# gsneha26/SegAlign

Hardware: AMD Instinct MI355X
Metric: Gbp query seeded+filtered+extended per sec (higher is better)
Workload: dtype int32

## Files before the change

### segalign_amd/csrc/extend.hip

```cpp
#include <atomic>
#include <cstdlib>

#include "kernels.h"
#include "kmer_dev.h"

namespace sa {

constexpr int EXT_THREADS = 256;
constexpr int NEG = -(1 << 26);
constexpr int DEAD = -(1 << 29);
constexpr uint64_t TERM_ALL = 0x4040404040404040ull;
constexpr uint32_t BIAS = SEQ_PAD;

__device__ __forceinline__ int f64_to_i32(double x) { return (int)x; }

enum : int { PH_RIGHT = 0, PH_LEFT = 1, PH_FIN = 2, PH_IDLE = 3 };

template <int CTRL, int ROW_MASK = 0xf, int BANK_MASK = 0xf>
__device__ __forceinline__ int dpp_mov(int old, int v) {
    return __builtin_amdgcn_update_dpp(old, v, CTRL, ROW_MASK, BANK_MASK, false);
}
__device__ __forceinline__ uint32_t wave_inclusive_sum(uint32_t v) {
    v += (uint32_t)dpp_mov<0x111>(0, (int)v);
    v += (uint32_t)dpp_mov<0x112>(0, (int)v);
// ... 410 lines not shown
        if (threadIdx.x < L2_NSUB) {
            raw = a.l2_count[threadIdx.x * L2_CNT_STRIDE];
            s_l2cnt[threadIdx.x & (SRC == SRC_CAND ? 0xFFFF : 0)] = min(raw, a.l2_cap);
        }
        __syncthreads();
        if (threadIdx.x <= L2_NSUB) {
            uint32_t pre = 0;
            for (int t = 0; t < (int)threadIdx.x; t++) pre += s_l2cnt[t & (SRC == SRC_CAND ? 0xFFFF : 0)];
            s_l2pre[threadIdx.x & (SRC == SRC_CAND ? 0xFFFF : 0)] = pre;
            if (blockIdx.x == 0 && threadIdx.x == L2_NSUB) *a.l2_total = pre;
        }
        if (blockIdx.x == 0 && threadIdx.x < L2_NSUB) {
            uint32_t mx = raw;
            for (int o = 32; o >= 1; o >>= 1) mx = max(mx, (uint32_t)__shfl_xor((int)mx, o, 64));
            if ((threadIdx.x & 63) == 0) atomicMax(a.l2_max, mx);
        }
    }
    __syncthreads();
    CandRec* stage = s_cand[threadIdx.x >> 6];
    int n_stage = 0;

    const int lane = threadIdx.x & 63;
    const unsigned long long lane_lt = (1ull << lane) - 1ull;
    const int xdrop = a.xdrop;
    const int fin_batch = a.fin_batch;
    const uint32_t long_cap = a.long_cap;

    const uint64_t total_hits = SRC == SRC_CAND ? (uint64_t)s_l2pre[SRC == SRC_CAND ? L2_NSUB : 0] : a.num_hits;
    const uint64_t num_buf = (total_hits + 63) >> 6;
    const uint64_t W = (uint64_t)gridDim.x * (PK_THREADS / 64);
    const uint64_t wid = (uint64_t)__builtin_amdgcn_readfirstlane((int)(blockIdx.x * (PK_THREADS / 64) + (threadIdx.x >> 6)));
    const uint64_t G = TD ? 1ull : W;
    const uint64_t buf_end = TD ? ((wid + 1) * num_buf) / W : num_buf;
    uint64_t cur_buf = TD ? (wid * num_buf) / W : wid;
    uint64_t nxt_buf = cur_buf + G;
    auto buf_count = [&](uint64_t b) -> int {
        if (b >= buf_end) return 0;
        uint64_t rem = total_hits - (b << 6);
        return rem >= 64 ? 64 : (int)rem;
    };
    TdCursor cursor = {0u, {0u, 0u, 0ull}, 0u};
    if (TD && cur_buf < buf_end) cursor.seek(a, lane, (uint32_t)(cur_buf << 6));
    uint32_t f_idx = 0;
    uint32_t f_known = 0, f_tm = 0, f_flags = 3;
    auto fetch = [&](uint64_t b, int cnt) -> Hit {
        Hit h = {0u, 0u};
        f_idx = (uint32_t)(b << 6) + (uint32_t)lane;
        if (SRC == SRC_HITS) {
            if (lane < cnt) h = a.hits[(b << 6) + lane];
        } else if (SRC == SRC_CAND) {
            if (lane < cnt) {
                const uint32_t g = (uint32_t)(b << 6) + (uint32_t)lane;
                uint32_t sl = 0;
#pragma unroll
                for (uint32_t step = L2_NSUB / 2; step >= 1; step >>= 1)
                    if (s_l2pre[(sl + step) & (SRC == SRC_CAND ? 0xFFFFu : 0u)] <= g) sl += step;
                const L2Rec c = a.l2_list[(size_t)sl * a.l2_cap + (g - s_l2pre[sl & (SRC == SRC_CAND ? 0xFFFFu : 0u)])];
                h.ref_loc = c.ref_loc;
                h.query_loc = c.query_loc;
                f_idx = c.hidx;
                f_known = c.meta & 0xFFFFu;
                f_flags = (c.meta >> 16) & 3u;
                const int t16 = (int)c.state >> 16;
                f_tm = ((uint32_t)t16 & 0xFFFFu) | ((uint32_t)(t16 + (int)(c.state & 0xFFFFu)) << 16);
            }
        } else if (cnt > 0) {
            uint64_t entry;
            uint32_t qp;
            cursor.locate(a, lane, (uint32_t)(b << 6), entry, qp);
            if (lane < cnt) {
                h.ref_loc = a.td_pos[entry] + a.seed_size;
                h.query_loc = qp + a.seed_size;
            }
        }
        return h;
    };
    int buf_cnt = buf_count(cur_buf), nxt_cnt = buf_count(nxt_buf), consumed = 0;
    Hit buf = fetch(cur_buf, buf_cnt);
    uint32_t buf_idx = f_idx, buf_known = f_known, buf_tm = f_tm, buf_flags = f_flags;
    Hit nxt = fetch(nxt_buf, nxt_cnt);
    uint32_t nxt_idx = f_idx, nxt_known = f_known, nxt_tm = f_tm, nxt_flags = f_flags;

    int phase = PH_FIN;
    bool has_hit = false, forward = false;
    uint32_t ref_loc = 0, query_loc = 0, hidx = 0;
    uint32_t walked = 0;
    uint4 h_tw = {0u, 0u, 0u, 0u}, h_qlo = {0u, 0u, 0u, 0u}, h_qhi = {0u, 0u, 0u, 0u};
    s16x2 T = {0, 0}, M = {0, 0};
    int bestR = 0, best = 0;
    bool left_known = false;
    int left_best = 0;

    for (;;) {
        if (phase < PH_FIN) {
            const bool left = phase == PH_LEFT;
            uint4 qlo, qhi, tw;
            if (left && walked == 0u) {
                qlo = h_qlo; qhi = h_qhi; tw = h_tw;
            } else {
                const int32_t qpos = left ? (int32_t)query_loc - (int32_t)walked : (int32_t)(query_loc + walked);
                const int32_t qbyte = left ? (qpos >> 1) - 32 : (qpos >> 1);
                const uint8_t* qp = a.query4 + (size_t)(qpos & 1) * a.query4_stride + qbyte;
                qlo = load16u(qp);
                qhi = load16u(qp + 16);
                const int32_t tpos = left ? (int32_t)ref_loc - (int32_t)walked : (int32_t)(ref_loc + walked);
                const int32_t tbyte = left ? (tpos >> 2) - 16 : (tpos >> 2);
                const bool fresh = !left && walked == 0u;
                const uint32_t jj0 = (uint32_t)(tbyte + PACK2_BIAS);
                const uint32_t line = (fresh ? jj0 - 16u : jj0) / (uint32_t)PACK2_PAYLOAD;
                const uint8_t* tp = a.ref2 + (size_t)(tpos & 3) * a.ref2_stride + (jj0 + 32u * line);
                tw = load16u(tp);
                if (fresh) {
                    h_tw = load16u(tp - 16);
                    h_qlo = load16u(qp - 32);
                    h_qhi = load16u(qp - 16);
                }
            }
            uint32_t tw0, tw1, tw2, tw3, qw0, qw1, qw2, qw3, qw4, qw5, qw6, qw7;
            if (left) {
                const uint32_t R = 0x00010203u, D = 0x88888888u;
                qw0 = __builtin_amdgcn_perm(0u, qhi.w, R) | D; qw1 = __builtin_amdgcn_perm(0u, qhi.z, R) | D;
                qw2 = __builtin_amdgcn_perm(0u, qhi.y, R) | D; qw3 = __builtin_amdgcn_perm(0u, qhi.x, R) | D;
                qw4 = __builtin_amdgcn_perm(0u, qlo.w, R) | D; qw5 = __builtin_amdgcn_perm(0u, qlo.z, R) | D;
                qw6 = __builtin_amdgcn_perm(0u, qlo.y, R) | D; qw7 = __builtin_amdgcn_perm(0u, qlo.x, R) | D;
                tw0 = __builtin_bitreverse32(tw.w); tw1 = __builtin_bitreverse32(tw.z);
                tw2 = __builtin_bitreverse32(tw.y); tw3 = __builtin_bitreverse32(tw.x);
            } else {
                qw0 = qlo.x; qw1 = qlo.y; qw2 = qlo.z; qw3 = qlo.w; qw4 = qhi.x; qw5 = qhi.y; qw6 = qhi.z; qw7 = qhi.w;
                tw0 = tw.x; tw1 = tw.y; tw2 = tw.z; tw3 = tw.w;
            }
            bool alive = true;
            int m = 0;
#pragma unroll
            for (int st = 0; st < 4; st++) {
                if (alive) {
                    const uint32_t td = st == 0 ? tw0 : st == 1 ? tw1 : st == 2 ? tw2 : tw3;
                    const uint32_t q0 = st == 0 ? qw0 : st == 1 ? qw2 : st == 2 ? qw4 : qw6;
                    const uint32_t q1 = st == 0 ? qw1 : st == 1 ? qw3 : st == 2 ? qw5 : qw7;
#pragma unroll
                    for (int j = 0; j < 8; j++) {
                        const uint32_t qd = j < 4 ? q0 : q1;
                        uint32_t qaddr;
                        switch (j & 3) {
                            case 0: asm("v_lshlrev_b32_sdwa %0, %1, %2 dst_sel:DWORD dst_unused:UNUSED_PAD src0_sel:DWORD src1_sel:BYTE_0" : "=v"(qaddr) : "v"(6), "v"(qd)); break;
                            case 1: asm("v_lshlrev_b32_sdwa %0, %1, %2 dst_sel:DWORD dst_unused:UNUSED_PAD src0_sel:DWORD src1_sel:BYTE_1" : "=v"(qaddr) : "v"(6), "v"(qd)); break;
                            case 2: asm("v_lshlrev_b32_sdwa %0, %1, %2 dst_sel:DWORD dst_unused:UNUSED_PAD src0_sel:DWORD src1_sel:BYTE_2" : "=v"(qaddr) : "v"(6), "v"(qd)); break;
                            default: asm("v_lshlrev_b32_sdwa %0, %1, %2 dst_sel:DWORD dst_unused:UNUSED_PAD src0_sel:DWORD src1_sel:BYTE_3" : "=v"(qaddr) : "v"(6), "v"(qd)); break;
                        }
                        const uint32_t rp = (td >> (4 * j)) & 15u;
                        const uint32_t addr = (rp << 2) | qaddr;
                        const s16x2 e = __builtin_bit_cast(s16x2, *reinterpret_cast<const uint32_t*>(reinterpret_cast<const char*>(s_pk) + addr));
                        const s16x2 Tb = T.yy;
                        T = __builtin_elementwise_add_sat(Tb, e);
                        M = __builtin_elementwise_max(M, T);
                    }
                    m = max((int)M.x, (int)M.y);
                    alive = (m - (int)T.y) <= xdrop;
                }
            }
            walked += 64;
            if (!alive) {
                if (!left) {
                    bestR = m;
                    if (SRC == SRC_CAND && left_known) {
                        best = left_best;
                        phase = PH_FIN;
                    } else {
                        phase = PH_LEFT;
                        walked = 0;
                        T = (s16x2){0, 0};
                        M = (s16x2){0, 0};
                    }
                } else {
                    best = m;
                    phase = PH_FIN;
                }
            } else if (walked + (uint32_t)(64 - CTX_R_BASES) >= long_cap) {
                forward = true;
                phase = PH_FIN;
            }
        }

        const unsigned long long fin = __ballot(phase == PH_FIN);
        const unsigned long long live = __ballot(phase < PH_FIN);
        if (fin != 0ull && (__popcll(fin) >= fin_batch || live == 0ull)) {
            bool cand = false;
            if (phase == PH_FIN && has_hit) cand = forward || bound_passes(a, bestR + best);
            {
                CandRec cr;
                cr.ref_loc = ref_loc; cr.query_loc = query_loc; cr.hidx = hidx;
                stage_append(stage, n_stage, cand, cr, a.cand_list, a.cand_count, a.cand_cap_recs, lane, lane_lt);
            }
            if (a.audit_list) {
                uint2 ar;
                ar.x = ref_loc; ar.y = query_loc;
                wave_append(phase == PH_FIN && has_hit && !cand, ar, a.audit_list, a.audit_count, a.audit_cap, lane, lane_lt);
            }
            unsigned long long need = fin;
            bool got = false;
            Hit mine = {0u, 0u};
            uint32_t mine_idx = 0, mine_known = 0, mine_tm = 0, mine_flags = 3;
            while (need != 0ull) {
                const int avail = buf_cnt - consumed;
                if (avail <= 0) {
                    if (nxt_cnt == 0) break;
                    buf = nxt;
                    buf_idx = nxt_idx;
                    buf_known = nxt_known; buf_tm = nxt_tm; buf_flags = nxt_flags;
                    buf_cnt = nxt_cnt;
                    cur_buf = nxt_buf;
                    consumed = 0;
                    nxt_buf += G;
                    nxt_cnt = buf_count(nxt_buf);
                    nxt = fetch(nxt_buf, nxt_cnt);
                    nxt_idx = f_idx;
                    nxt_known = f_known; nxt_tm = f_tm; nxt_flags = f_flags;
                    continue;
                }
                const int rank = __popcll(need & lane_lt);
                const bool take = ((need >> lane) & 1ull) && rank < avail;
                const int src = (consumed + rank) & 63;
                const uint32_t hr = (uint32_t)__shfl((int)buf.ref_loc, src, 64);
                const uint32_t hq = (uint32_t)__shfl((int)buf.query_loc, src, 64);
                const uint32_t hi = SRC == SRC_CAND ? (uint32_t)__shfl((int)buf_idx, src, 64) : (uint32_t)(cur_buf << 6) + (uint32_t)src;
                uint32_t hk = 0, ht = 0, hf = 3;
                if (SRC == SRC_CAND) {
                    hk = (uint32_t)__shfl((int)buf_known, src, 64);
                    ht = (uint32_t)__shfl((int)buf_tm, src, 64);
                    hf = (uint32_t)__shfl((int)buf_flags, src, 64);
                }
                if (take) {
                    mine.ref_loc = hr;
                    mine.query_loc = hq;
                    mine_idx = hi;
                    mine_known = hk; mine_tm = ht; mine_flags = hf;
                    got = true;
                }
                consumed += min(__popcll(need), avail);
                need &= ~__ballot(take);
            }
            if (phase == PH_FIN) {
                forward = false;
                if (got) {
                    has_hit = true;
                    ref_loc = mine.ref_loc;
                    query_loc = mine.query_loc;
                    hidx = mine_idx;
                    bestR = 0;
                    best = 0;
                    bool skip = false;
                    if (a.rm) skip = !(ref_loc >= a.rm_win_start && ref_loc <= a.rm_win_end);
                    left_known = false;
                    if (skip || ref_loc > a.ref_len || query_loc > a.query_len) {
                        phase = PH_FIN;
                    } else if (SRC == SRC_CAND && mine_flags == 0u) {
                        bestR = (int)mine_known;
                        best = (int)mine_tm;
                        phase = PH_FIN;
                    } else if (SRC == SRC_CAND && mine_flags == 2u) {
                        bestR = (int)mine_known;
                        phase = PH_LEFT;
                        walked = (uint32_t)CTX_L_BASES + a.left_skip;
                        const short t16 = (short)(mine_tm & 0xFFFFu), m16 = (short)(mine_tm >> 16);
                        T = (s16x2){t16, t16};
                        M = (s16x2){m16, m16};
                    } else {
                        phase = PH_RIGHT;
                        walked = 0;
                        T = (s16x2){0, 0};
                        M = (s16x2){0, 0};
                        if (SRC == SRC_CAND && mine_flags == 1u) {
                            left_known = true;
                            left_best = (int)mine_known;
                            if (a.l2_right_state) {
                                walked = (uint32_t)CTX_R_BASES;
                                const short t16 = (short)(mine_tm & 0xFFFFu), m16 = (short)(mine_tm >> 16);
                                T = (s16x2){t16, t16};
                                M = (s16x2){m16, m16};
                            }
                        }
                    }
                } else {
                    has_hit = false;
                    phase = PH_IDLE;
                }
            }
        }
        if (__ballot(phase != PH_IDLE) == 0ull) break;
    }
    stage_flush(stage, n_stage, a.cand_list, a.cand_count, a.cand_cap_recs, lane);
}

constexpr int CTX_THREADS = 1024;
constexpr int CTX_THREADS_MAX = 1024;
constexpr int CTX_STAGE_FLUSH = 32;
constexpr int CTX_STAGE_CAP = CTX_STAGE_FLUSH - 1 + 64 + 1;
constexpr int CLS_TAB = 4096;
constexpr int CLS_TAIL = 256;
constexpr int CLS_LDS_DWORDS = CLS_TAB + CLS_TAIL;
constexpr bool CLS_TRACK_DROP = true;
constexpr int CLS_TILE = 64;
constexpr int CLS_WIN_DWORDS = 5;
constexpr uint32_t CLS_WIN_SPAN = CLS_TILE - CLS_WIN_DWORDS;
constexpr int CLS_TILE_BYTES = CLS_TILE * (int)sizeof(TdRec) + 2 * CLS_TILE * 4;

__device__ __forceinline__ void cls_table_init(uint32_t* __restrict__ s_cls, const int* cls, int nthreads) {
    const int c0 = cls[0], c1 = cls[1], c2 = cls[2], c3 = cls[3];
    for (int i = threadIdx.x; i < CLS_TAB + CLS_TAIL; i += nthreads) {
        const int nb = i < CLS_TAB ? 6 : 4;
        const int f = i < CLS_TAB ? i : i - CLS_TAB;
        int sum = 0, mx = 0;
        for (int k = 0; k < nb; k++) {
            const int x = (f >> (2 * k)) & 3;
            sum += x == 0 ? c0 : x == 1 ? c1 : x == 2 ? c2 : c3;
            mx = max(mx, sum);
        }
        s_cls[i] = ((uint32_t)sum << 16) | ((uint32_t)(sum - mx) & 0xFFFFu);
    }
}

template <int O>
__device__ __forceinline__ uint32_t cls_field_addr(uint32_t w0, uint32_t w1) {
    constexpr uint32_t MASK = 0x3FFCu;
    if (O + 12 <= 32) return O >= 2 ? ((w0 >> (O - 2)) & MASK) : ((w0 << (2 - O)) & MASK);
    return __builtin_amdgcn_alignbit(w1, w0, (uint32_t)(O - 2)) & MASK;
}

__device__ __forceinline__ uint32_t mul24(uint32_t x, uint32_t s_uniform) {
    uint32_t r;
    asm("v_mul_u32_u24 %0, %1, %2" : "=v"(r) : "s"(s_uniform), "v"(x));
    return r;
}

__device__ __forceinline__ void cls_step(const uint32_t* __restrict__ s_tab, uint32_t addr, uint32_t& P, uint32_t& W) {
    const uint32_t e = *reinterpret_cast<const uint32_t*>(reinterpret_cast<const char*>(s_tab) + addr);
    asm("v_pk_add_i16 %0, %1, %2 op_sel:[0,1] op_sel_hi:[1,1]" : "=v"(P) : "v"(P), "v"(e));
    asm("v_min_i16_sdwa %0, %0, %1 dst_sel:WORD_0 dst_unused:UNUSED_PRESERVE src0_sel:WORD_0 src1_sel:WORD_0" : "+v"(P) : "v"(e));
    if (CLS_TRACK_DROP) {
        typedef short s16x2 __attribute__((ext_vector_type(2)));
        W = __builtin_bit_cast(uint32_t, __builtin_elementwise_min(__builtin_bit_cast(s16x2, W), __builtin_bit_cast(s16x2, P)));
    }
}

__device__ __forceinline__ uint32_t cls_seed_state(const ExtendArgs& a) {
    const int cmax = max(max(a.cls[0], a.cls[1]), max(a.cls[2], a.cls[3]));
    return (uint32_t)((int)a.left_skip * max(cmax, 0)) << 16;
}

template <bool ONE_COPY>
__global__ __launch_bounds__(CTX_THREADS_MAX, 8) void extend_filter_cls_kernel(ExtendArgs a) {
    __shared__ __attribute__((aligned(16))) uint32_t s_cls[CLS_LDS_DWORDS];
    extern __shared__ __attribute__((aligned(16))) L2Rec s_l2_dyn[];
    cls_table_init(s_cls, a.cls, (int)blockDim.x);
    __syncthreads();
    const uint32_t* __restrict__ s_tail = s_cls + CLS_TAB;
    L2Rec* stage = s_l2_dyn + (threadIdx.x >> 6) * CTX_STAGE_CAP;
    int n_stage = 0;
    const int lane = threadIdx.x & 63;
    const int xdrop = a.xdrop;
    const uint4* __restrict__ ctx = reinterpret_cast<const uint4*>(a.td_ctx);
    const uint32_t seed_state = cls_seed_state(a);

    const uint64_t num_buf = (a.num_hits + 63) >> 6;
    const uint64_t n_chunks = (a.num_hits + TD_CHUNK_HITS - 1) / TD_CHUNK_HITS;
    const uint64_t W = (uint64_t)gridDim.x * (blockDim.x >> 6);
    const uint64_t wid = (uint64_t)__builtin_amdgcn_readfirstlane((int)(blockIdx.x * (blockDim.x >> 6) + (threadIdx.x >> 6)));
    const uint64_t c_lo = (wid * n_chunks) / W, c_hi = ((wid + 1) * n_chunks) / W;
    const uint64_t b_lo = c_lo * (TD_CHUNK_HITS / 64);
    const uint64_t b_hi = min(c_hi * (TD_CHUNK_HITS / 64), num_buf);
    if (b_lo >= b_hi) return;
    const uint32_t my_sub = (uint32_t)wid & (uint32_t)(L2_NSUB - 1);
    L2Rec* __restrict__ my_list = a.l2_list + (size_t)my_sub * a.l2_cap;
    uint32_t* __restrict__ my_count = a.l2_count + my_sub * L2_CNT_STRIDE;
    typedef const uint64_t __attribute__((address_space(4))) * HeadPtr;
    HeadPtr head = (HeadPtr)a.td_bits;
    const uint32_t stride16 = (uint32_t)(a.q2_stride >> 4) & 0xFFFFFFu;
    uint32_t cbefore;
    auto locate = [&](uint64_t B) -> uint32_t {
        const uint64_t Bs = B >> 1;
        const uint32_t idx = __builtin_amdgcn_mbcnt_hi((uint32_t)(Bs >> 32), __builtin_amdgcn_mbcnt_lo((uint32_t)Bs, cbefore - 1u + (uint32_t)(B & 1ull)));
        cbefore += (uint32_t)__builtin_popcountll(B);
        return idx;
    };
    struct Stage {
        uint4 c0, tl;
        uint32_t q[7];
        uint32_t query_loc;
    };
    auto merge_q = [&](Stage& S, uint32_t qr0, uint32_t qr1, uint32_t qr2, uint32_t qr3, uint32_t ql0, uint32_t ql1, uint32_t ql2, uint32_t ql3) {
        S.q[0] = qr0; S.q[1] = qr1; S.q[2] = qr2;
        S.q[3] = (qr3 & 0xFFFu) | (ql0 << 12);
        S.q[4] = __builtin_amdgcn_alignbit(ql1, ql0, 20);
        S.q[5] = __builtin_amdgcn_alignbit(ql2, ql1, 20);
        S.q[6] = __builtin_amdgcn_alignbit(ql3, ql2, 20);
    };
    uint64_t w0, w1, w2;
    uint64_t wc = 0;
    TdRec hnext;
    typedef uint32_t u32x4 __attribute__((ext_vector_type(4)));
    typedef u32x4 __attribute__((address_space(3))) * LdsU4;
    typedef uint32_t __attribute__((address_space(3))) * LdsU32;
    LdsU4 s_td = nullptr;
    LdsU32 s_qr = nullptr, s_ql = nullptr;
    uint32_t td0 = 0, dr0 = 0, dl0 = 0;
    const uint32_t q2_last = (uint32_t)(a.q2_stride >> 2) - 1u;
    if (ONE_COPY) {
        char* tiles = reinterpret_cast<char*>(s_l2_dyn) + (size_t)(blockDim.x >> 6) * (CTX_STAGE_CAP * sizeof(L2Rec)) + (size_t)(threadIdx.x >> 6) * CLS_TILE_BYTES;
        s_td = (LdsU4)tiles;
        s_qr = (LdsU32)(tiles + CLS_TILE * sizeof(TdRec));
        s_ql = s_qr + CLS_TILE;
    }
    auto rare_lane = [&]() -> uint32_t {
        uint32_t l = (uint32_t)lane;
        asm volatile("" : "+v"(l));
        return l;
    };
    auto tile_td = [&](uint32_t base) {
        const uint32_t l = rare_lane();
        const TdRec r = a.td_rec[min(base + l, a.td_m)];
        __builtin_amdgcn_wave_barrier();
        s_td[l] = u32x4{r.prefix, r.qpos, (uint32_t)r.off, (uint32_t)(r.off >> 32)};
        __builtin_amdgcn_wave_barrier();
        td0 = base;
    };
    auto tile_q = [&](uint32_t own_dword, uint32_t other_dword) {
        const uint32_t nr = own_dword, nl = other_dword > CLS_WIN_SPAN ? other_dword - CLS_WIN_SPAN : 0u;
        const uint32_t l = rare_lane();
        const uint32_t vr = reinterpret_cast<const uint32_t*>(a.q2_own)[min(nr + l, q2_last)];
        const uint32_t vl = reinterpret_cast<const uint32_t*>(a.q2_other)[min(nl + l, q2_last)];
        __builtin_amdgcn_wave_barrier();
        s_qr[l] = vr;
        s_ql[l] = vl;
        __builtin_amdgcn_wave_barrier();
        dr0 = nr;
        dl0 = nl;
    };
    auto advance_map = [&](uint64_t b_req) {
        if (ONE_COPY) wc = w0;
        else hnext = a.td_rec[locate(w0)];
        w0 = w1;
        w1 = w2;
        w2 = head[b_req + 4];
    };
    auto request = [&](uint64_t b, Stage& S) {
        if (ONE_COPY) {
            const uint32_t idx = locate(wc);
            if (__builtin_expect(__ballot(idx - td0 >= (uint32_t)CLS_TILE) != 0ull, 0)) tile_td((uint32_t)__builtin_amdgcn_readfirstlane((int)idx));
            const u32x4 r = s_td[idx - td0];
            hnext.prefix = r.x;
            hnext.qpos = r.y;
            hnext.off = (uint64_t)r.z | ((uint64_t)r.w << 32);
        }
        const uint64_t entry = hnext.off + (uint64_t)((uint32_t)(b << 6) + (uint32_t)lane - hnext.prefix);
        S.c0 = ctx[2 * entry];
        S.tl = ctx[2 * entry + 1];
        const uint32_t query_loc = hnext.qpos + a.seed_size;
        S.query_loc = query_loc;
        const uint32_t lp = a.query_len - query_loc + a.left_skip;
        if (ONE_COPY) {
            uint4 t, u;
            uint32_t t4, u4;
            const uint32_t dr = query_loc >> 4, dl = lp >> 4;
            const uint32_t sr = (query_loc & 15u) << 1, sl = (lp & 15u) << 1;
            bool tiled = true;
            if (__builtin_expect(__ballot(dr - dr0 > CLS_WIN_SPAN || dl - dl0 > CLS_WIN_SPAN) != 0ull, 0)) {
                tile_q((uint32_t)__builtin_amdgcn_readfirstlane((int)dr), (uint32_t)__builtin_amdgcn_readfirstlane((int)dl));
                tiled = __ballot(dr - dr0 > CLS_WIN_SPAN || dl - dl0 > CLS_WIN_SPAN) == 0ull;
            }
            if (tiled) {
                const LdsU32 rp = s_qr + (dr - dr0), lq = s_ql + (dl - dl0);
                t = make_uint4(rp[0], rp[1], rp[2], rp[3]);
                t4 = rp[4];
                u = make_uint4(lq[0], lq[1], lq[2], lq[3]);
                u4 = lq[4];
            } else {
                const uint8_t* rpp = a.q2_own + (dr << 2);
                __builtin_memcpy(&t, __builtin_assume_aligned(rpp, 4), 16);
                __builtin_memcpy(&t4, __builtin_assume_aligned(rpp + 16, 4), 4);
                const uint8_t* lpp = a.q2_other + (dl << 2);
                __builtin_memcpy(&u, __builtin_assume_aligned(lpp, 4), 16);
                __builtin_memcpy(&u4, __builtin_assume_aligned(lpp + 16, 4), 4);
                __builtin_amdgcn_s_waitcnt(0x0F70);
            }
            merge_q(S, __builtin_amdgcn_alignbit(t.y, t.x, sr), __builtin_amdgcn_alignbit(t.z, t.y, sr), __builtin_amdgcn_alignbit(t.w, t.z, sr),
                    __builtin_amdgcn_alignbit(t4, t.w, sr), __builtin_amdgcn_alignbit(u.y, u.x, sl), __builtin_amdgcn_alignbit(u.z, u.y, sl),
                    __builtin_amdgcn_alignbit(u.w, u.z, sl), __builtin_amdgcn_alignbit(u4, u.w, sl));
        } else {
            const uint32_t po = (mul24(query_loc & 15u, stride16) << 4) + ((query_loc >> 4) << 2);
            uint4 t, u;
            __builtin_memcpy(&t, __builtin_assume_aligned(a.q2_own + po, 4), 16);
            const uint32_t qo = (mul24(lp & 15u, stride16) << 4) + ((lp >> 4) << 2);
            __builtin_memcpy(&u, __builtin_assume_aligned(a.q2_other + qo, 4), 16);
            merge_q(S, t.x, t.y, t.z, t.w, u.x, u.y, u.z, u.w);
        }
    };
    auto score = [&](uint64_t b, const Stage& S) {
        const bool valid = (b << 6) + (uint64_t)lane < a.num_hits;
        const uint32_t query_loc = S.query_loc;
        const uint32_t ref_loc = S.c0.x + a.seed_size;
        bool skip = !valid;
        if (a.rm) skip = skip || !(ref_loc >= a.rm_win_start && ref_loc <= a.rm_win_end);
        const uint32_t x0 = S.c0.y ^ S.q[0], x1 = S.c0.z ^ S.q[1], x2 = S.c0.w ^ S.q[2], x3 = S.tl.x ^ S.q[3], x4 = S.tl.y ^ S.q[4],
                       x5 = S.tl.z ^ S.q[5], x6 = S.tl.w ^ S.q[6];
        uint32_t P = 0, Wd = 0;
        cls_step(s_cls, cls_field_addr<0>(x0, x1), P, Wd);
        cls_step(s_cls, cls_field_addr<12>(x0, x1), P, Wd);
        cls_step(s_cls, cls_field_addr<24>(x0, x1), P, Wd);
        cls_step(s_cls, cls_field_addr<4>(x1, x2), P, Wd);
        cls_step(s_cls, cls_field_addr<16>(x1, x2), P, Wd);
        cls_step(s_cls, cls_field_addr<28>(x1, x2), P, Wd);
        cls_step(s_cls, cls_field_addr<8>(x2, x3), P, Wd);
        cls_step(s_cls, cls_field_addr<20>(x2, x3), P, Wd);
        cls_step(s_cls, cls_field_addr<0>(x3, x4), P, Wd);
        const bool r_alive = (int)(short)((CLS_TRACK_DROP ? Wd : P) & 0xFFFFu) >= -xdrop;
        const int bestR = ((int)P >> 16) - (int)(short)(P & 0xFFFFu);
        const uint32_t PR = P;
        P = seed_state; Wd = 0;
        cls_step(s_cls, cls_field_addr<12>(x3, x4), P, Wd);
        cls_step(s_cls, cls_field_addr<24>(x3, x4), P, Wd);
        cls_step(s_cls, cls_field_addr<4>(x4, x5), P, Wd);
        cls_step(s_cls, cls_field_addr<16>(x4, x5), P, Wd);
        cls_step(s_cls, cls_field_addr<28>(x4, x5), P, Wd);
        cls_step(s_cls, cls_field_addr<8>(x5, x6), P, Wd);
        cls_step(s_cls, cls_field_addr<20>(x5, x6), P, Wd);
        cls_step(s_cls, cls_field_addr<0>(x6, 0u), P, Wd);
        cls_step(s_cls, cls_field_addr<12>(x6, 0u), P, Wd);
        cls_step(s_tail, (x6 >> 22) & 0x3FCu, P, Wd);
        const bool l_alive = (int)(short)((CLS_TRACK_DROP ? Wd : P) & 0xFFFFu) >= -xdrop;
        const int bestL = ((int)P >> 16) - (int)(short)(P & 0xFFFFu);
        const bool fwd = !skip && (r_alive || l_alive || bound_passes(a, bestR + bestL));
        const unsigned long long fm = __ballot(fwd);
        if (fm) {
            L2Rec cr;
            cr.ref_loc = ref_loc;
            cr.query_loc = query_loc;
            cr.hidx = (uint32_t)(b << 6) + (uint32_t)lane;
            const uint32_t fl = (r_alive ? 1u : 0u) | (l_alive ? 2u : 0u);
            const uint32_t Ps = (fl == 1u && a.l2_right_state) ? PR : P;
            cr.state = (Ps & 0xFFFF0000u) | ((0u - Ps) & 0xFFFFu);
            cr.meta = (uint32_t)(r_alive ? bestL : bestR) | ((fl ? fl : 3u) << 16);
            const uint32_t rank = __builtin_amdgcn_mbcnt_hi((uint32_t)(fm >> 32), __builtin_amdgcn_mbcnt_lo((uint32_t)fm, 0u));
            if (fwd) stage[n_stage + (int)rank] = cr;
            n_stage += __popcll(fm);
            __builtin_amdgcn_wave_barrier();
            if (n_stage >= CTX_STAGE_FLUSH) {
                const int k = n_stage < 64 ? n_stage : 64;
                stage_flush(stage, k, my_list, my_count, a.l2_cap, lane);
                const int rest = n_stage - k;
                L2Rec tmp = cr;
                if (lane < rest) tmp = stage[k + lane];
                __builtin_amdgcn_wave_barrier();
                if (lane < rest) stage[lane] = tmp;
                __builtin_amdgcn_wave_barrier();
                n_stage = rest;
            }
        }
        if (a.audit_list) {
            uint2 ar;
            ar.x = ref_loc;
            ar.y = query_loc;
            wave_append(valid && !skip && !fwd, ar, a.audit_list, a.audit_count, a.audit_cap, lane, (1ull << rare_lane()) - 1ull);
        }
    };
    Stage SA, SB;
    {
        const uint64_t h0 = head[b_lo];
        w0 = head[b_lo + 1];
        w1 = head[b_lo + 2];
        w2 = head[b_lo + 3];
        cbefore = a.td_chunk[c_lo] + 1u - (uint32_t)(h0 & 1ull);
        if (ONE_COPY) {
            const uint32_t i0 = a.td_chunk[c_lo];
            const uint32_t ql0 = a.td_rec[i0].qpos + a.seed_size;
            wc = h0;
            tile_td(i0);
            tile_q(ql0 >> 4, (a.query_len - ql0 + a.left_skip) >> 4);
        } else {
            hnext = a.td_rec[locate(h0)];
        }
        request(b_lo, SA);
        advance_map(b_lo);
    }
    uint64_t b = b_lo;
    for (; b + 1 < b_hi; b += 2) {
        request(b + 1, SB);
        advance_map(b + 1);
        score(b, SA);
        request(b + 2, SA);
        advance_map(b + 2);
        score(b + 1, SB);
    }
    if (b < b_hi) score(b, SA);
    stage_flush(stage, n_stage, my_list, my_count, a.l2_cap, lane);
}

__device__ __forceinline__ int rfl(int v) { return __builtin_amdgcn_readfirstlane(v); }

template <bool COUNT_EXAMINED, bool XDROP_NONNEG>
__device__ __forceinline__ void wave_extend_exact(const ExtendArgs& a, const int* __restrict__ s_tab,
                                                  const uint8_t* __restrict__ R8b, const uint8_t* __restrict__ Qb, int lane,
                                                  uint32_t ref_loc, uint32_t query_loc, int& bestR, int& bposR, int& bestL,
                                                  int& boffL, unsigned long long& examined) {
    const int xdrop = a.xdrop;
    bestR = 0; bposR = -1; bestL = 0; boffL = 0;
    bool skip = false;
    if (a.rm) skip = !(ref_loc >= a.rm_win_start && ref_loc <= a.rm_win_end);
    if (skip) bposR = 0;
    for (int side = skip ? 2 : 0; side < 2; side++) {
        const bool left = side == 1;
        const uint32_t lim = left ? min(ref_loc, query_loc)
                                  : ((ref_loc < a.ref_len && query_loc < a.query_len)
                                         ? min(a.ref_len - ref_loc, a.query_len - query_loc) : 0u);
        uint32_t k0 = left ? 1u : 0u;
        int score_in = 0, best_in = 0, bpos_in = left ? 0 : -1;
        for (;;) {
            const uint32_t k = k0 + 8u * (uint32_t)lane;
            const int64_t rem64 = left ? (int64_t)lim - (int64_t)k + 1 : (int64_t)lim - (int64_t)k;
            const int remaining = rem64 > 8 ? 8 : (rem64 < 0 ? 0 : (int)rem64);
            uint64_t x = 0;
            if (remaining > 0) {
                const uint32_t roff = left ? ref_loc + BIAS - k - 7u : ref_loc + BIAS + k;
                const uint32_t qoff = left ? query_loc + BIAS - k - 7u : query_loc + BIAS + k;
                x = load8u(R8b + roff) | load8u(Qb + qoff);
                if (left) x = __builtin_bswap64(x);
            }
            if (remaining < 8) x |= (remaining <= 0) ? TERM_ALL : (TERM_ALL << (8 * remaining));
            uint32_t run = 0;
            int mx = INT32_MIN, amx = 0;
            {
                const uint32_t xlo = (uint32_t)x, xhi = (uint32_t)(x >> 32);
#pragma unroll
                for (int j = 0; j < 8; j++) {
                    const uint32_t w = j < 4 ? xlo : xhi;
                    run += (uint32_t)s_tab[(w >> (8 * (j & 3))) & 0xffu];
                    const bool up = (int)run > mx;
                    amx = up ? j : amx;
                    mx = up ? (int)run : mx;
                }
            }
            const uint32_t inc = wave_inclusive_sum(run);
            const int base = (int)((uint32_t)score_in + inc - run);
            int mv = (int)((uint32_t)base + (uint32_t)mx), mp = (int)(k + (uint32_t)amx);
            wave_inclusive_max(mv, mp);
            int ev = dpp_mov<0x138>(INT32_MIN, mv);
            int ep = dpp_mov<0x138>(0, mp);
            if (best_in >= ev) { ev = best_in; ep = bpos_in; }
            int score = base, best = ev, bpos = ep;
            uint32_t ex_step = 0;
            chunk8_exact<COUNT_EXAMINED, XDROP_NONNEG>(s_tab, x, k, xdrop, score, best, bpos, ex_step);
            const unsigned long long dm = __ballot(score < (DEAD >> 1));
            if (dm) {
                const int f = __ffsll((long long)dm) - 1;
                best_in = __builtin_amdgcn_readlane(best, f);
                bpos_in = __builtin_amdgcn_readlane(bpos, f);
                if (COUNT_EXAMINED && lane <= f) examined += ex_step;
                break;
            }
            if (COUNT_EXAMINED) examined += ex_step;
            score_in = __builtin_amdgcn_readlane(score, 63);
            best_in = __builtin_amdgcn_readlane(best, 63);
            bpos_in = __builtin_amdgcn_readlane(bpos, 63);
            k0 += 512u;
        }
        if (!left) { bestR = best_in; bposR = bpos_in; }
        else { bestL = best_in; boffL = bpos_in; }
    }
}

struct ExactStage {
    HspRec* st_out;
    EntRec* st_ent;
    int n_out, n_ent;
};

__device__ __forceinline__ void wave_finalize(const ExtendArgs& a, ExactStage& st, int lane, uint32_t ref_loc, uint32_t query_loc,
                                              uint32_t seg, int bestR, int bposR, int bestL, int boffL) {
    const int total = bestR + bestL, extent = bposR + boffL;
    const int cls = classify(a, total);
    if (!cls) return;
    if (cls == 1) {
        if (lane == 0) st.st_out[st.n_out] = make_rec(a, ref_loc, query_loc, boffL, extent, total, seg);
        st.n_out++;
        __builtin_amdgcn_wave_barrier();
        if (st.n_out == 64) { stage_flush(st.st_out, 64, a.out, a.out_count, a.out_cap, lane); st.n_out = 0; __builtin_amdgcn_wave_barrier(); }
    } else {
        if (lane == 0) {
            EntRec er;
            er.ref_loc = ref_loc; er.query_loc = query_loc; er.bposR = bposR; er.boffL = boffL; er.total = total; er.seg = seg;
            st.st_ent[st.n_ent] = er;
        }
        st.n_ent++;
        __builtin_amdgcn_wave_barrier();
        if (st.n_ent == 64) { stage_flush(st.st_ent, 64, a.ent_list, a.ent_count, a.ent_cap_recs, lane); st.n_ent = 0; __builtin_amdgcn_wave_barrier(); }
    }
}

#define EXACT_KERNEL_PROLOGUE()                                                                            \
    __shared__ int s_tab[128];                                                                             \
    __shared__ HspRec s_out[EXT_THREADS / 64][64];                                                         \
    __shared__ EntRec s_ent[EXT_THREADS / 64][64];                                                         \
    if (threadIdx.x < 128) s_tab[threadIdx.x] = threadIdx.x < 64 ? a.sub_mat[threadIdx.x] : NEG;           \
    __syncthreads();                                                                                       \
    ExactStage st = {s_out[threadIdx.x >> 6], s_ent[threadIdx.x >> 6], 0, 0};                             \
    const int lane = threadIdx.x & 63;                                                                     \
    const uint8_t* __restrict__ R8b = a.ref8 - BIAS;                                                       \
    const uint8_t* __restrict__ Qb = a.query - BIAS;                                                       \
    const uint32_t n_cand = min(*a.cand_count, a.cand_cap_recs);                                           \
    const uint32_t G = gridDim.x * (EXT_THREADS / 64);                                                     \
    SEG_TABLE()                                                                                            \
    unsigned long long examined = 0;

#define EXACT_KERNEL_EPILOGUE()                                                                            \
    stage_flush(st.st_out, st.n_out, a.out, a.out_count, a.out_cap, lane);                                 \
    stage_flush(st.st_ent, st.n_ent, a.ent_list, a.ent_count, a.ent_cap_recs, lane);                       \
    if (COUNT_EXAMINED) {                                                                                  \
        unsigned long long v = examined;                                                                   \
        for (int off = 32; off > 0; off >>= 1) v += __shfl_down(v, off, 64);                               \
        if (lane == 0 && v) atomicAdd(a.examined, v);                                                      \
    }

template <bool COUNT_EXAMINED, bool XDROP_NONNEG>
__global__ __launch_bounds__(EXT_THREADS) void extend_exact_kernel(ExtendArgs a) {
    EXACT_KERNEL_PROLOGUE()
    if (a.chain_cap && n_cand <= a.chain_cap) return;
    for (uint32_t i = blockIdx.x * (EXT_THREADS / 64) + (threadIdx.x >> 6); i < n_cand; i += G) {
        const CandRec cr = a.cand_list[i];
        const uint32_t ref_loc = (uint32_t)rfl((int)cr.ref_loc), query_loc = (uint32_t)rfl((int)cr.query_loc);
        const uint32_t hidx = (uint32_t)rfl((int)cr.hidx);
        int bestR, bposR, bestL, boffL;
        wave_extend_exact<COUNT_EXAMINED, XDROP_NONNEG>(a, s_tab, R8b, Qb, lane, ref_loc, query_loc, bestR, bposR, bestL, boffL, examined);
        wave_finalize(a, st, lane, ref_loc, query_loc, seg_of(a, s_seg, hidx), bestR, bposR, bestL, boffL);
    }
    EXACT_KERNEL_EPILOGUE()
}

constexpr uint32_t CHAIN_GAP_MAX = 256;
constexpr uint32_t CHAIN_WALK_EXTRA = 96;

constexpr uint32_t CHAIN_BUCKETS_MIN = 16384, CHAIN_BUCKETS_MAX = 262144;
constexpr uint32_t CHAIN_SORT_MAX = 4096;

constexpr uint32_t CHAIN_QSHIFT = 9;
__device__ __forceinline__ uint32_t chain_bucket_of(uint32_t buckets, uint32_t seg, const CandRec& c) {
    const uint32_t diag = c.ref_loc - c.query_loc;
    return (((diag * 2654435761u) ^ ((c.query_loc >> CHAIN_QSHIFT) * 0x85EBCA6Bu) ^ (seg * 0x9E3779B1u)) >> 14) & (buckets - 1u);
}
__device__ __forceinline__ uint32_t chain_buckets_of(const ExtendArgs& a, uint32_t n) {
    if (a.chain_buckets) return a.chain_buckets;
    const uint32_t want = n / a.chain_bucket_target;
    uint32_t b = CHAIN_BUCKETS_MIN;
    while (b < CHAIN_BUCKETS_MAX && b < want) b <<= 1;
    return b;
}
__device__ __forceinline__ bool chain_range(const ExtendArgs& a, uint32_t& first, uint32_t& n) {
    const uint32_t total = min(*a.cand_count, a.cand_cap_recs);
    if (a.cand_sliced) {
        first = a.cand_first;
        n = total > first ? min(total - first, a.chain_cap) : 0u;
        return n > 0;
    }
    first = 0;
    n = total;
    return total <= a.chain_cap;
}

template <bool DOWN>
__device__ __forceinline__ uint32_t wave_bucket_add(uint32_t* __restrict__ counters, bool active, uint32_t b, uint32_t& base) {
    const int lane = threadIdx.x & 63;
    uint32_t rank = 0, k = 0;
    int my_leader = lane;
    unsigned long long todo = __ballot(active);
    while (todo) {
        const int leader = __ffsll((long long)todo) - 1;
        const uint32_t b0 = (uint32_t)__builtin_amdgcn_readlane((int)b, leader);
        const unsigned long long same = __ballot(active && b == b0) & todo;
        if ((same >> lane) & 1ull) {
            my_leader = leader;
            rank = (uint32_t)__popcll(same & ((1ull << lane) - 1ull));
            k = (uint32_t)__popcll(same);
        }
        todo &= ~same;
    }
    uint32_t got = 0;
    if (active && lane == my_leader) got = DOWN ? atomicSub(&counters[b], k) - k : atomicAdd(&counters[b], k);
    base = (uint32_t)__shfl((int)got, my_leader, 64);
    return rank;
}

__global__ __launch_bounds__(256) void chain_count_kernel(ExtendArgs a) {
    uint32_t first, n;
    if (!chain_range(a, first, n)) return;
    SEG_TABLE()
    const uint32_t B = chain_buckets_of(a, n);
    const uint32_t stride = gridDim.x * blockDim.x;
    const uint32_t rounds = (n + stride - 1) / stride;
    for (uint32_t r = 0; r < rounds; r++) {
        const uint32_t i = r * stride + blockIdx.x * blockDim.x + threadIdx.x;
        uint32_t b = 0;
        if (i < n) {
            const CandRec c = a.cand_list[first + i];
            b = chain_bucket_of(B, seg_of(a, s_seg, c.hidx), c);
        }
        uint32_t base;
        wave_bucket_add<false>(a.chain_bucket_cnt, i < n, b, base);
    }
}

constexpr uint32_t CHAIN_SCAN_THREADS = 1024, CHAIN_SCAN_TILE = CHAIN_SCAN_THREADS * 4;
__global__ __launch_bounds__(CHAIN_SCAN_THREADS) void chain_scan_kernel(ExtendArgs a) {
    __shared__ uint32_t s_tile[CHAIN_SCAN_THREADS / 64], s_front[CHAIN_SCAN_THREADS / 64];
    uint32_t first, n;
    if (!chain_range(a, first, n)) return;
    const uint32_t B = chain_buckets_of(a, n);
    const uint32_t t0 = blockIdx.x * CHAIN_SCAN_TILE;
    if (t0 >= B) return;
    const uint4* cnt4 = reinterpret_cast<const uint4*>(a.chain_bucket_cnt);
    uint4* start4 = reinterpret_cast<uint4*>(a.chain_bucket_start);
    const int lane = threadIdx.x & 63, wave = threadIdx.x >> 6;
    uint32_t front = 0;
    for (uint32_t q = threadIdx.x; q < (t0 >> 2); q += CHAIN_SCAN_THREADS) {
        const uint4 f = cnt4[q];
        front += f.x + f.y + f.z + f.w;
    }
    const uint4 v = cnt4[(t0 >> 2) + threadIdx.x];
    const uint32_t sum = v.x + v.y + v.z + v.w;
    uint32_t inc = sum;
#pragma unroll
    for (int off = 1; off < 64; off <<= 1) {
        const uint32_t t = __shfl_up(inc, off, 64);
        if (lane >= off) inc += t;
    }
#pragma unroll
    for (int off = 32; off >= 1; off >>= 1) front += __shfl_xor(front, off, 64);
    if (lane == 63) {
        s_tile[wave] = inc;
        s_front[wave] = front;
    }
    __syncthreads();
    uint32_t base = inc - sum;
    for (int w = 0; w < (int)(CHAIN_SCAN_THREADS / 64); w++) base += s_front[w] + (w < wave ? s_tile[w] : 0u);
    start4[(t0 >> 2) + threadIdx.x] = make_uint4(base, base + v.x, base + v.x + v.y, base + v.x + v.y + v.z);
    if (t0 + CHAIN_SCAN_TILE >= B && threadIdx.x == CHAIN_SCAN_THREADS - 1) a.chain_bucket_start[B] = base + sum;
}

__global__ __launch_bounds__(256) void chain_scatter_kernel(ExtendArgs a) {
    uint32_t first, n;
    if (!chain_range(a, first, n)) return;
    SEG_TABLE()
    const uint32_t B = chain_buckets_of(a, n);
    const uint32_t stride = gridDim.x * blockDim.x;
    const uint32_t rounds = (n + stride - 1) / stride;
    for (uint32_t r = 0; r < rounds; r++) {
        const uint32_t i = r * stride + blockIdx.x * blockDim.x + threadIdx.x;
        uint32_t b = 0;
        CandRec c = {0u, 0u, 0u};
        if (i < n) {
            c = a.cand_list[first + i];
            b = chain_bucket_of(B, seg_of(a, s_seg, c.hidx), c);
        }
        uint32_t base;
        const uint32_t rank = wave_bucket_add<true>(a.chain_bucket_cnt, i < n, b, base);
        if (i < n) a.chain_tmp[a.chain_bucket_start[b] + base + rank] = c;
    }
}

constexpr uint32_t CHAIN_SORT_GROUP = 8;

template <bool XDROP_NONNEG>
__device__ __forceinline__ bool chain_is_run_head(const ExtendArgs& a, const uint64_t* __restrict__ s_seg, const int* __restrict__ s_tab, const uint8_t* __restrict__ R8b,
                                                  const uint8_t* __restrict__ Qb, const CandRec& c, const CandRec& pc) {
    if (!((c.ref_loc - c.query_loc) == (pc.ref_loc - pc.query_loc) && c.query_loc > pc.query_loc && seg_of(a, s_seg, c.hidx) == seg_of(a, s_seg, pc.hidx)))
        return true;
    const uint32_t g = c.query_loc - pc.query_loc;
    if (g > CHAIN_GAP_MAX) return true;
    const uint32_t lim = min(c.ref_loc, c.query_loc);
    int score = 0, best = 0, bpos = 0;
    uint32_t ex = 0;
    for (uint32_t k = 1; k <= g + CHAIN_WALK_EXTRA; k += 8) {
        const int64_t rem64 = (int64_t)lim - (int64_t)k + 1;
// ... 283 lines not shown
```

Baseline: 1.312.

## Cache per-seed-position query strings and ctx base pointers in LDS slots

```diff
diff --git a/segalign_amd/csrc/extend.hip b/segalign_amd/csrc/extend.hip
--- a/segalign_amd/csrc/extend.hip
+++ b/segalign_amd/csrc/extend.hip
@@ -736,7 +736,10 @@
 constexpr int CLS_TILE = 64;
 constexpr int CLS_WIN_DWORDS = 5;
 constexpr uint32_t CLS_WIN_SPAN = CLS_TILE - CLS_WIN_DWORDS;
-constexpr int CLS_TILE_BYTES = CLS_TILE * (int)sizeof(TdRec) + 2 * CLS_TILE * 4;
+constexpr int CLS_POS_SLOTS = 32;
+constexpr int CLS_POS_SLOT_BYTES = 40;
+constexpr int CLS_TILE_BYTES = CLS_POS_SLOTS * CLS_POS_SLOT_BYTES + 2 * CLS_TILE * 4;
+static_assert((CLS_POS_SLOTS & (CLS_POS_SLOTS - 1)) == 0 && CLS_POS_SLOTS <= 64 && CLS_TILE_BYTES % 16 == 0 && CLS_TILE_BYTES <= 2112, "position tile");
 
 __device__ __forceinline__ void cls_table_init(uint32_t* __restrict__ s_cls, const int* cls, int nthreads) {
     const int c0 = cls[0], c1 = cls[1], c2 = cls[2], c3 = cls[3];
@@ -821,27 +824,33 @@
         uint32_t q[7];
         uint32_t query_loc;
     };
-    auto merge_q = [&](Stage& S, uint32_t qr0, uint32_t qr1, uint32_t qr2, uint32_t qr3, uint32_t ql0, uint32_t ql1, uint32_t ql2, uint32_t ql3) {
-        S.q[0] = qr0; S.q[1] = qr1; S.q[2] = qr2;
-        S.q[3] = (qr3 & 0xFFFu) | (ql0 << 12);
-        S.q[4] = __builtin_amdgcn_alignbit(ql1, ql0, 20);
-        S.q[5] = __builtin_amdgcn_alignbit(ql2, ql1, 20);
-        S.q[6] = __builtin_amdgcn_alignbit(ql3, ql2, 20);
+    auto merge_q = [&](uint32_t (&q)[7], uint32_t qr0, uint32_t qr1, uint32_t qr2, uint32_t qr3, uint32_t ql0, uint32_t ql1, uint32_t ql2, uint32_t ql3) {
+        q[0] = qr0; q[1] = qr1; q[2] = qr2;
+        q[3] = (qr3 & 0xFFFu) | (ql0 << 12);
+        q[4] = __builtin_amdgcn_alignbit(ql1, ql0, 20);
+        q[5] = __builtin_amdgcn_alignbit(ql2, ql1, 20);
+        q[6] = __builtin_amdgcn_alignbit(ql3, ql2, 20);
     };
     uint64_t w0, w1, w2;
     uint64_t wc = 0;
     TdRec hnext;
     typedef uint32_t u32x4 __attribute__((ext_vector_type(4)));
+    typedef uint32_t u32x2 __attribute__((ext_vector_type(2)));
     typedef u32x4 __attribute__((address_space(3))) * LdsU4;
+    typedef u32x2 __attribute__((address_space(3))) * LdsU2;
     typedef uint32_t __attribute__((address_space(3))) * LdsU32;
-    LdsU4 s_td = nullptr;
+    typedef const u32x4 __attribute__((address_space(1))) * GlobU4;
+    LdsU4 s_pa = nullptr, s_pb = nullptr;
+    LdsU2 s_pc = nullptr;
     LdsU32 s_qr = nullptr, s_ql = nullptr;
     uint32_t td0 = 0, dr0 = 0, dl0 = 0;
     const uint32_t q2_last = (uint32_t)(a.q2_stride >> 2) - 1u;
     if (ONE_COPY) {
         char* tiles = reinterpret_cast<char*>(s_l2_dyn) + (size_t)(blockDim.x >> 6) * (CTX_STAGE_CAP * sizeof(L2Rec)) + (size_t)(threadIdx.x >> 6) * CLS_TILE_BYTES;
-        s_td = (LdsU4)tiles;
-        s_qr = (LdsU32)(tiles + CLS_TILE * sizeof(TdRec));
+        s_pa = (LdsU4)tiles;
+        s_pb = s_pa + CLS_POS_SLOTS;
+        s_pc = (LdsU2)(s_pb + CLS_POS_SLOTS);
+        s_qr = (LdsU32)(s_pc + CLS_POS_SLOTS);
         s_ql = s_qr + CLS_TILE;
     }
     auto rare_lane = [&]() -> uint32_t {
@@ -849,15 +858,7 @@
         asm volatile("" : "+v"(l));
         return l;
     };
-    auto tile_td = [&](uint32_t base) {
-        const uint32_t l = rare_lane();
-        const TdRec r = a.td_rec[min(base + l, a.td_m)];
-        __builtin_amdgcn_wave_barrier();
-        s_td[l] = u32x4{r.prefix, r.qpos, (uint32_t)r.off, (uint32_t)(r.off >> 32)};
-        __builtin_amdgcn_wave_barrier();
-        td0 = base;
-    };
-    auto tile_q = [&](uint32_t own_dword, uint32_t other_dword) {
+    auto tile_q = [&](uint32_t own_dword, uint32_t other_dword) __attribute__((always_inline)) {
         const uint32_t nr = own_dword, nl = other_dword > CLS_WIN_SPAN ? other_dword - CLS_WIN_SPAN : 0u;
         const uint32_t l = rare_lane();
         const uint32_t vr = reinterpret_cast<const uint32_t*>(a.q2_own)[min(nr + l, q2_last)];
@@ -869,6 +870,50 @@
         dr0 = nr;
         dl0 = nl;
     };
+    auto make_string = [&](uint32_t query_loc, uint32_t (&q)[7]) __attribute__((always_inline)) {
+        const uint32_t lp = a.query_len - query_loc + a.left_skip;
+        const uint32_t dr = query_loc >> 4, dl = lp >> 4;
+        const uint32_t sr = (query_loc & 15u) << 1, sl = (lp & 15u) << 1;
+        if (__ballot(dr - dr0 > CLS_WIN_SPAN || dl - dl0 > CLS_WIN_SPAN) != 0ull)
+            tile_q((uint32_t)__builtin_amdgcn_readfirstlane((int)dr), (uint32_t)__builtin_amdgcn_readfirstlane((int)dl));
+        uint4 t, u;
+        uint32_t t4, u4;
+        if (!(dr - dr0 > CLS_WIN_SPAN || dl - dl0 > CLS_WIN_SPAN)) {
+            const LdsU32 rp = s_qr + (dr - dr0), lq = s_ql + (dl - dl0);
+            t = make_uint4(rp[0], rp[1], rp[2], rp[3]);
+            t4 = rp[4];
+            u = make_uint4(lq[0], lq[1], lq[2], lq[3]);
+            u4 = lq[4];
+        } else {
+            const uint8_t* rpp = a.q2_own + (dr << 2);
+            __builtin_memcpy(&t, __builtin_assume_aligned(rpp, 4), 16);
+            __builtin_memcpy(&t4, __builtin_assume_aligned(rpp + 16, 4), 4);
+            const uint8_t* lpp = a.q2_other + (dl << 2);
+            __builtin_memcpy(&u, __builtin_assume_aligned(lpp, 4), 16);
+            __builtin_memcpy(&u4, __builtin_assume_aligned(lpp + 16, 4), 4);
+            __builtin_amdgcn_s_waitcnt(0x0F70);
+        }
+        merge_q(q, __builtin_amdgcn_alignbit(t.y, t.x, sr), __builtin_amdgcn_alignbit(t.z, t.y, sr), __builtin_amdgcn_alignbit(t.w, t.z, sr),
+                __builtin_amdgcn_alignbit(t4, t.w, sr), __builtin_amdgcn_alignbit(u.y, u.x, sl), __builtin_amdgcn_alignbit(u.z, u.y, sl),
+                __builtin_amdgcn_alignbit(u.w, u.z, sl), __builtin_amdgcn_alignbit(u4, u.w, sl));
+    };
+    auto stream_base = [&](const TdRec& r) -> uint64_t { return reinterpret_cast<uint64_t>(ctx) + ((r.off - (uint64_t)r.prefix) << 5); };
+    auto tile_pos = [&](uint32_t base) __attribute__((always_inline)) {
+        const uint32_t l = rare_lane();
+        const TdRec r = a.td_rec[min(base + (l & (uint32_t)(CLS_POS_SLOTS - 1)), a.td_m)];
+        const uint32_t query_loc = r.qpos + a.seed_size;
+        uint32_t q[7];
+        make_string(query_loc, q);
+        const uint64_t rb = stream_base(r);
+        __builtin_amdgcn_wave_barrier();
+        if (l < (uint32_t)CLS_POS_SLOTS) {
+            s_pa[l] = u32x4{q[0], q[1], q[2], q[3]};
+            s_pb[l] = u32x4{q[4], q[5], q[6], query_loc};
+            s_pc[l] = u32x2{(uint32_t)rb, (uint32_t)(rb >> 32)};
+        }
+        __builtin_amdgcn_wave_barrier();
+        td0 = base;
+    };
     auto advance_map = [&](uint64_t b_req) {
         if (ONE_COPY) wc = w0;
         else hnext = a.td_rec[locate(w0)];
@@ -879,11 +924,33 @@
     auto request = [&](uint64_t b, Stage& S) {
         if (ONE_COPY) {
             const uint32_t idx = locate(wc);
-            if (__builtin_expect(__ballot(idx - td0 >= (uint32_t)CLS_TILE) != 0ull, 0)) tile_td((uint32_t)__builtin_amdgcn_readfirstlane((int)idx));
-            const u32x4 r = s_td[idx - td0];
-            hnext.prefix = r.x;
-            hnext.qpos = r.y;
-            hnext.off = (uint64_t)r.z | ((uint64_t)r.w << 32);
+            bool slots = true;
+            if (__builtin_expect(__ballot(idx - td0 >= (uint32_t)CLS_POS_SLOTS) != 0ull, 0)) {
+                tile_pos((uint32_t)__builtin_amdgcn_readfirstlane((int)idx));
+                slots = __ballot(idx - td0 >= (uint32_t)CLS_POS_SLOTS) == 0ull;
+            }
+            uint64_t rb;
+            if (__builtin_expect(slots, 1)) {
+                const uint32_t k = idx - td0;
+                const u32x4 qa = s_pa[k], qb = s_pb[k];
+                const u32x2 pc = s_pc[k];
+                S.q[0] = qa.x; S.q[1] = qa.y; S.q[2] = qa.z; S.q[3] = qa.w;
+                S.q[4] = qb.x; S.q[5] = qb.y; S.q[6] = qb.z;
+                S.query_loc = qb.w;
+                rb = (uint64_t)pc.x | ((uint64_t)pc.y << 32);
+            } else {
+                const TdRec r = a.td_rec[min(idx, a.td_m)];
+                S.query_loc = r.qpos + a.seed_size;
+                make_string(S.query_loc, S.q);
+                rb = stream_base(r);
+                __builtin_amdgcn_s_waitcnt(0x0F70);
+            }
+            const uint64_t at = ((uint64_t)(uint32_t)(b << 6) << 5) | (uint64_t)((uint32_t)lane << 5);
+            const GlobU4 rec = (GlobU4)(rb + at);
+            const u32x4 c0 = rec[0], tl = rec[1];
+            S.c0 = make_uint4(c0.x, c0.y, c0.z, c0.w);
+            S.tl = make_uint4(tl.x, tl.y, tl.z, tl.w);
+            return;
         }
         const uint64_t entry = hnext.off + (uint64_t)((uint32_t)(b << 6) + (uint32_t)lane - hnext.prefix);
         S.c0 = ctx[2 * entry];
@@ -891,42 +958,12 @@
         const uint32_t query_loc = hnext.qpos + a.seed_size;
         S.query_loc = query_loc;
         const uint32_t lp = a.query_len - query_loc + a.left_skip;
-        if (ONE_COPY) {
-            uint4 t, u;
-            uint32_t t4, u4;
-            const uint32_t dr = query_loc >> 4, dl = lp >> 4;
-            const uint32_t sr = (query_loc & 15u) << 1, sl = (lp & 15u) << 1;
-            bool tiled = true;
-            if (__builtin_expect(__ballot(dr - dr0 > CLS_WIN_SPAN || dl - dl0 > CLS_WIN_SPAN) != 0ull, 0)) {
-                tile_q((uint32_t)__builtin_amdgcn_readfirstlane((int)dr), (uint32_t)__builtin_amdgcn_readfirstlane((int)dl));
-                tiled = __ballot(dr - dr0 > CLS_WIN_SPAN || dl - dl0 > CLS_WIN_SPAN) == 0ull;
-            }
-            if (tiled) {
-                const LdsU32 rp = s_qr + (dr - dr0), lq = s_ql + (dl - dl0);
-                t = make_uint4(rp[0], rp[1], rp[2], rp[3]);
-                t4 = rp[4];
-                u = make_uint4(lq[0], lq[1], lq[2], lq[3]);
-                u4 = lq[4];
-            } else {
-                const uint8_t* rpp = a.q2_own + (dr << 2);
-                __builtin_memcpy(&t, __builtin_assume_aligned(rpp, 4), 16);
-                __builtin_memcpy(&t4, __builtin_assume_aligned(rpp + 16, 4), 4);
-                const uint8_t* lpp = a.q2_other + (dl << 2);
-                __builtin_memcpy(&u, __builtin_assume_aligned(lpp, 4), 16);
-                __builtin_memcpy(&u4, __builtin_assume_aligned(lpp + 16, 4), 4);
-                __builtin_amdgcn_s_waitcnt(0x0F70);
-            }
-            merge_q(S, __builtin_amdgcn_alignbit(t.y, t.x, sr), __builtin_amdgcn_alignbit(t.z, t.y, sr), __builtin_amdgcn_alignbit(t.w, t.z, sr),
-                    __builtin_amdgcn_alignbit(t4, t.w, sr), __builtin_amdgcn_alignbit(u.y, u.x, sl), __builtin_amdgcn_alignbit(u.z, u.y, sl),
-                    __builtin_amdgcn_alignbit(u.w, u.z, sl), __builtin_amdgcn_alignbit(u4, u.w, sl));
-        } else {
-            const uint32_t po = (mul24(query_loc & 15u, stride16) << 4) + ((query_loc >> 4) << 2);
-            uint4 t, u;
-            __builtin_memcpy(&t, __builtin_assume_aligned(a.q2_own + po, 4), 16);
-            const uint32_t qo = (mul24(lp & 15u, stride16) << 4) + ((lp >> 4) << 2);
-            __builtin_memcpy(&u, __builtin_assume_aligned(a.q2_other + qo, 4), 16);
-            merge_q(S, t.x, t.y, t.z, t.w, u.x, u.y, u.z, u.w);
-        }
+        const uint32_t po = (mul24(query_loc & 15u, stride16) << 4) + ((query_loc >> 4) << 2);
+        uint4 t, u;
+        __builtin_memcpy(&t, __builtin_assume_aligned(a.q2_own + po, 4), 16);
+        const uint32_t qo = (mul24(lp & 15u, stride16) << 4) + ((lp >> 4) << 2);
+        __builtin_memcpy(&u, __builtin_assume_aligned(a.q2_other + qo, 4), 16);
+        merge_q(S.q, t.x, t.y, t.z, t.w, u.x, u.y, u.z, u.w);
     };
     auto score = [&](uint64_t b, const Stage& S) {
         const bool valid = (b << 6) + (uint64_t)lane < a.num_hits;
@@ -1007,8 +1044,8 @@
             const uint32_t i0 = a.td_chunk[c_lo];
             const uint32_t ql0 = a.td_rec[i0].qpos + a.seed_size;
             wc = h0;
-            tile_td(i0);
             tile_q(ql0 >> 4, (a.query_len - ql0 + a.left_skip) >> 4);
+            tile_pos(i0);
         } else {
             hnext = a.td_rec[locate(h0)];
         }
```

New measurement: 1.341, median of 6. 1.02x the previous value.
